# andres-fr/realtime-pose-estimation

Measured on AMD Instinct MI355X. Metric: images/sec at 640x640 (HRNet-w48 fwd+decode), higher is better.
Workload: dtype f16 (fp32 accumulate, fp32 BatchNorm; fp32 NCHW in/out); 1 GPU; configs[2]: batch=32 per GPU, 640x640, half-wrapper teacher forward + decode of 17 keypoint channels, weights W0 (seeded random); batch_per_gpu=32, people_per_batch_rank0=960

## Files before the change

realtime-pose-estimation_amd/csrc/conv_block.hip:

```cpp
#include <type_traits>

#include "rtpe_common.h"

namespace rtpe {

typedef _Float16 half8 __attribute__((ext_vector_type(8)));
typedef _Float16 half4 __attribute__((ext_vector_type(4)));
typedef float float4v __attribute__((ext_vector_type(4)));
typedef float float2v __attribute__((ext_vector_type(2)));
typedef _Float16 half2v __attribute__((ext_vector_type(2)));

__device__ __forceinline__ half4 bn_round(const float4v v, const float4v al, const float4v be) {
  const half2v h0 = __builtin_convertvector(float2v{v[0], v[1]}, half2v);
  const half2v h1 = __builtin_convertvector(float2v{v[2], v[3]}, half2v);
  float r0 = __builtin_fmaf((float)h0[0], al[0], be[0]);
  float r1 = __builtin_fmaf((float)h0[1], al[1], be[1]);
  float r2 = __builtin_fmaf((float)h1[0], al[2], be[2]);
  float r3 = __builtin_fmaf((float)h1[1], al[3], be[3]);
  asm volatile("" : "+v"(r0), "+v"(r1), "+v"(r2), "+v"(r3));
  const half2v o0 = __builtin_convertvector(float2v{r0, r1}, half2v), o1 = __builtin_convertvector(float2v{r2, r3}, half2v);
  return half4{o0[0], o0[1], o1[0], o1[1]};
}
typedef short short8 __attribute__((ext_vector_type(8)));
typedef short short4v __attribute__((ext_vector_type(4)));

namespace {

constexpr int kTH = 6, kTW = 32;
constexpr int kMH = kTH + 2, kMW = kTW + 2;
constexpr int kXH = kTH + 4, kXW = kTW + 4;
constexpr int kPS = 96;
constexpr int kMT = 3;
constexpr int kNT1 = 5, kNT2 = 3;
constexpr int kWaves = 4, kLoad = 3;
constexpr int kKH = 7;
constexpr int kWSlot = kMT * kKH * 1024;
constexpr int kXBytes = kXH * kXW * kPS;
constexpr int kMidBytes = kMH * kMW * kPS;
constexpr int kRowB = kMT * 32 + 16;
constexpr int kNIT = (kNT2 * 16 * 6 + 63) / 64;
constexpr int kLds = 3 * kWSlot + 2 * kXBytes + kMidBytes;

#define RTPE_BBARRIER()                         \
  do {                                          \
    asm volatile("" ::: "memory");              \
    __builtin_amdgcn_s_barrier();               \
    asm volatile("" ::: "memory");              \
  } while (0)

typedef __attribute__((address_space(3))) void* lds_ptr_t;

}

struct BlockArgs {
  const _Float16* x;
  _Float16* y;
  const _Float16* w1;
  const _Float16* w2;
  const float* ab1;
  const float* ab2;
  int N, H, W, in_ld, out_ld;
  int tiles_x, tiles_y;
  FastDiv div_tiles_x, div_tiles_xy;
  int x_bytes;
  int ablate;
};

__global__ void __launch_bounds__((kWaves + kLoad) * 64) conv_block_kernel(const BlockArgs a) {
  extern __shared__ __attribute__((aligned(16))) char smem[];
  char* const wring = smem;
  char* const xt = smem + 3 * kWSlot;
  char* const mid = xt + 2 * kXBytes;
  const int tid = threadIdx.x;
  const int lane = tid & 63;
  const int wv = __builtin_amdgcn_readfirstlane(tid >> 6);

  const int n_tiles = a.N * a.tiles_x * a.tiles_y;
  const int G = (int)(gridDim.x >> 3), xcd = (int)(blockIdx.x & 7), jw = (int)(blockIdx.x >> 3);
  const int per_xcd = (n_tiles + 7) >> 3;
  const int t_begin = xcd * per_xcd;
  const int tiles_xcd = min(per_xcd, n_tiles - t_begin);
  const int U = jw < tiles_xcd ? (tiles_xcd - jw + G - 1) / G : 0;
  if (U == 0) return;
  const uint32_t tiles_xy = (uint32_t)(a.tiles_x * a.tiles_y);
  auto unit_origin = [&](int u, uint32_t* n, int* py0, int* px0) __attribute__((always_inline)) {
    uint32_t t = (uint32_t)(t_begin + jw + u * G);
    *n = fdiv(t, a.div_tiles_xy);
    t -= *n * tiles_xy;
    const uint32_t tyi = fdiv(t, a.div_tiles_x);
    *py0 = (int)tyi * kTH;
    *px0 = (int)(t - tyi * a.tiles_x) * kTW;
  };

  if (wv == kWaves) {
    __amdgpu_buffer_rsrc_t r1 = __builtin_amdgcn_make_buffer_rsrc(const_cast<_Float16*>(a.w1), 0, 2 * kWSlot, 0x00020000);
    __amdgpu_buffer_rsrc_t r2 = __builtin_amdgcn_make_buffer_rsrc(const_cast<_Float16*>(a.w2), 0, 2 * kWSlot, 0x00020000);
    const int voff = lane * 16;
    auto issue = [&](int q) __attribute__((always_inline)) {
      const int i = q & 3;
      char* dst = wring + (q % 3) * kWSlot;
      const int src = (i & 1) * kWSlot;
      if (i < 2) {
#pragma unroll
        for (int p = 0; p < kMT * kKH; ++p)
          __builtin_amdgcn_raw_ptr_buffer_load_lds(r1, (lds_ptr_t)(dst + p * 1024), 16, voff, src + p * 1024, 0, 0);
      } else {
#pragma unroll
        for (int p = 0; p < kMT * kKH; ++p)
          __builtin_amdgcn_raw_ptr_buffer_load_lds(r2, (lds_ptr_t)(dst + p * 1024), 16, voff, src + p * 1024, 0, 0);
      }
    };
    const int Q = 4 * U;
    issue(0);
    issue(1);
    for (int q = 0; q < Q; ++q) {
      if (q + 1 < Q) asm volatile("s_waitcnt vmcnt(%0)" ::"n"(kMT * kKH) : "memory");
      else asm volatile("s_waitcnt vmcnt(0)" ::: "memory");
      RTPE_BBARRIER();
      if (q + 2 < Q) issue(q + 2);
      if ((q & 3) == 3) RTPE_BBARRIER();
    }
    asm volatile("s_waitcnt vmcnt(0)" ::: "memory");
    return;
  }

  if (wv > kWaves) {
    const int jl = wv - kWaves - 1;
    __amdgpu_buffer_rsrc_t rsrc = __builtin_amdgcn_make_buffer_rsrc(const_cast<_Float16*>(a.x), 0, a.x_bytes, 0x00020000);
    constexpr int rowslots = kXW * 6;
    auto issue = [&](int u) __attribute__((always_inline)) {
      uint32_t n;
      int py0, px0;
      unit_origin(u, &n, &py0, &px0);
      const int iy0 = py0 - 2, ix0 = px0 - 2;
      uint32_t voff[4];
#pragma unroll
      for (int k = 0; k < 4; ++k) {
        const int q = k * 64 + lane;
        const int hx = q / 6, sl = q - hx * 6;
        const int ix = ix0 + hx;
        voff[k] = (unsigned)ix < (unsigned)a.W ? (uint32_t)(ix * a.in_ld + sl * 8) * 2u : 0x80000000u;
      }
      char* buf = xt + (u & 1) * kXBytes;
      const int img_row0 = (int)n * a.H;
      for (int r = jl * (kXH / 2); r < (jl + 1) * (kXH / 2); ++r) {
        const int iy = iy0 + r;
        const bool row_ok = (unsigned)iy < (unsigned)a.H;
        const int soff = row_ok ? (img_row0 + iy) * a.W * a.in_ld * 2 : 0;
        char* dst = buf + r * (kXW * kPS);
#pragma unroll
        for (int k = 0; k < 4; ++k)
          if (k * 64 + lane < rowslots)
            __builtin_amdgcn_raw_ptr_buffer_load_lds(rsrc, (lds_ptr_t)(dst + k * 1024), 16,
                                                     (int)(row_ok ? voff[k] : 0x80000000u), soff, 0, 0);
      }
    };
    issue(0);
    for (int u = 0; u < U; ++u) {
      asm volatile("s_waitcnt vmcnt(0)" ::: "memory");
      RTPE_BBARRIER();
      if (u + 1 < U) issue(u + 1);
      RTPE_BBARRIER();
      RTPE_BBARRIER();
      RTPE_BBARRIER();
      RTPE_BBARRIER();
    }
    asm volatile("s_waitcnt vmcnt(0)" ::: "memory");
    return;
  }

  const int r = lane & 15, g = lane >> 4;
  int toff1[2 * kKH], toff2[2 * kKH];
#pragma unroll
  for (int k = 0; k < 2 * kKH; ++k) {
    int kk = k * 32 + g * 8;
    if (kk >= 9 * 48) kk -= 9 * 48;
    const int tap = kk / 48, c = kk - tap * 48;
    const int ty = tap / 3, tx = tap - ty * 3;
    toff1[k] = (ty * kXW + tx) * kPS + c * 2;
    toff2[k] = (ty * kMW + tx) * kPS + c * 2;
  }
  int pix1[kNT1], pix2[kNT2];
#pragma unroll
  for (int nt = 0; nt < kNT1; ++nt) {
    int p = (wv * kNT1 + nt) * 16 + r;
    p = p < kMH * kMW ? p : kMH * kMW - 1;
    const int my = p / kMW, mx = p - my * kMW;
    pix1[nt] = (my * kXW + mx) * kPS;
  }
#pragma unroll
  for (int nt = 0; nt < kNT2; ++nt) {
    const int p = (wv * kNT2 + nt) * 16 + r;
    pix2[nt] = ((p >> 5) * kMW + (p & 31)) * kPS;
  }
  float4v al1[kMT], be1[kMT], al2[kMT], be2[kMT];
#pragma unroll
  for (int m = 0; m < kMT; ++m) {
    const int c4 = m * 16 + g * 4;
    al1[m] = *reinterpret_cast<const float4v*>(a.ab1 + c4);
    be1[m] = *reinterpret_cast<const float4v*>(a.ab1 + 48 + c4);
    al2[m] = *reinterpret_cast<const float4v*>(a.ab2 + c4);
    be2[m] = *reinterpret_cast<const float4v*>(a.ab2 + 48 + c4);
  }
#pragma unroll
  for (int m = 0; m < kMT; ++m) asm volatile("" ::"v"(al1[m]), "v"(be1[m]), "v"(al2[m]), "v"(be2[m]));

  int eoff[kNIT], xoff[kNIT], epos[kNIT];
#pragma unroll
  for (int it = 0; it < kNIT; ++it) {
    int c = it * 64 + lane;
    const bool exists = c < kNT2 * 16 * 6;
    c = exists ? c : 0;
    const int pw = c / 6, slot = c - pw * 6;
    const int p = wv * kNT2 * 16 + pw;
    const int oy = p >> 5, ox = p & 31;
    eoff[it] = pw * kRowB + slot * 16;
    xoff[it] = ((oy + 2) * kXW + ox + 2) * kPS + slot * 16;
    epos[it] = ((exists ? oy : 0x7fff) << 16) | (ox << 8) | (slot * 16);
  }
  int wsel = 0;
  for (int u = 0; u < U; ++u) {
    uint32_t n;
    int py0, px0;
    unit_origin(u, &n, &py0, &px0);
    const char* xb = xt + (u & 1) * kXBytes;

    float4v acc1[kMT][kNT1];
#pragma unroll
    for (int m = 0; m < kMT; ++m)
#pragma unroll
      for (int nt = 0; nt < kNT1; ++nt) acc1[m][nt] = float4v{0.f, 0.f, 0.f, 0.f};
#pragma unroll
    for (int h = 0; h < 2; ++h) {
      RTPE_BBARRIER();
      const char* wl = wring + wsel * kWSlot + lane * 16;
      wsel = wsel == 2 ? 0 : wsel + 1;
      half8 af[2][kMT], bf[2][kNT1];
#pragma unroll
      for (int m = 0; m < kMT; ++m) af[0][m] = *reinterpret_cast<const half8*>(wl + m * 1024);
#pragma unroll
      for (int nt = 0; nt < kNT1; ++nt) bf[0][nt] = *reinterpret_cast<const half8*>(xb + pix1[nt] + toff1[h * kKH]);
#pragma unroll
      for (int kk = 0; kk < kKH; ++kk) {
        const int cur = kk & 1, nxt = cur ^ 1;
        if (kk + 1 < kKH) {
#pragma unroll
          for (int m = 0; m < kMT; ++m) af[nxt][m] = *reinterpret_cast<const half8*>(wl + ((kk + 1) * kMT + m) * 1024);
#pragma unroll
          for (int nt = 0; nt < kNT1; ++nt)
            bf[nxt][nt] = *reinterpret_cast<const half8*>(xb + pix1[nt] + toff1[h * kKH + kk + 1]);
        }
#pragma unroll
        for (int m = 0; m < kMT; ++m)
#pragma unroll
          for (int nt = 0; nt < kNT1; ++nt)
            acc1[m][nt] = __builtin_amdgcn_mfma_f32_16x16x32_f16(af[cur][m], bf[cur][nt], acc1[m][nt], 0, 0, 0);
        if (kk + 1 < kKH) {
#pragma unroll
          for (int i = 0; i < (kMT + kNT1 + 3) / 4; ++i) {
            __builtin_amdgcn_sched_group_barrier(0x008, 1, 0);
            __builtin_amdgcn_sched_group_barrier(0x002, 4, 0);
            __builtin_amdgcn_sched_group_barrier(0x100, 4, 0);
          }
        }
        __builtin_amdgcn_sched_barrier(0);
      }
    }
    {
      int lane_e = lane;
      asm volatile("" : "+v"(lane_e));
      const int re = lane_e & 15, ge = lane_e >> 4;
#pragma unroll
      for (int nt = 0; nt < kNT1; ++nt) {
        const int p = (wv * kNT1 + nt) * 16 + re;
        const int my = p / kMW, mx = p - my * kMW;
        const int iy = py0 - 1 + my, ix = px0 - 1 + mx;
        const bool inside = (unsigned)iy < (unsigned)a.H && (unsigned)ix < (unsigned)a.W;
#pragma unroll
        for (int m = 0; m < kMT; ++m) {
          const half4 o_bn = bn_round(acc1[m][nt], al1[m], be1[m]);
          short4v b = __builtin_bit_cast(short4v, o_bn);
          b = b & ~(b >> 15);
          if (!inside) b = b ^ b;
          if (p < kMH * kMW)
            *reinterpret_cast<short4v*>(mid + p * kPS + m * 32 + ge * 8) = b;
        }
      }
      asm volatile("s_waitcnt lgkmcnt(0)" ::: "memory");
    }

    float4v acc2[kMT][kNT2];
#pragma unroll
    for (int m = 0; m < kMT; ++m)
#pragma unroll
      for (int nt = 0; nt < kNT2; ++nt) acc2[m][nt] = float4v{0.f, 0.f, 0.f, 0.f};
#pragma unroll
    for (int h = 0; h < 2; ++h) {
      RTPE_BBARRIER();
      const char* wl = wring + wsel * kWSlot + lane * 16;
      wsel = wsel == 2 ? 0 : wsel + 1;
      half8 af[2][kMT], bf[2][kNT2];
#pragma unroll
      for (int m = 0; m < kMT; ++m) af[0][m] = *reinterpret_cast<const half8*>(wl + m * 1024);
#pragma unroll
      for (int nt = 0; nt < kNT2; ++nt) bf[0][nt] = *reinterpret_cast<const half8*>(mid + pix2[nt] + toff2[h * kKH]);
#pragma unroll
      for (int kk = 0; kk < kKH; ++kk) {
        const int cur = kk & 1, nxt = cur ^ 1;
        if (kk + 1 < kKH) {
#pragma unroll
          for (int m = 0; m < kMT; ++m) af[nxt][m] = *reinterpret_cast<const half8*>(wl + ((kk + 1) * kMT + m) * 1024);
#pragma unroll
          for (int nt = 0; nt < kNT2; ++nt)
            bf[nxt][nt] = *reinterpret_cast<const half8*>(mid + pix2[nt] + toff2[h * kKH + kk + 1]);
        }
#pragma unroll
        for (int m = 0; m < kMT; ++m)
#pragma unroll
          for (int nt = 0; nt < kNT2; ++nt)
            acc2[m][nt] = __builtin_amdgcn_mfma_f32_16x16x32_f16(af[cur][m], bf[cur][nt], acc2[m][nt], 0, 0, 0);
        if (kk + 1 < kKH) {
#pragma unroll
          for (int i = 0; i < (kMT + kNT2 + 3) / 4; ++i) {
            __builtin_amdgcn_sched_group_barrier(0x008, 1, 0);
            __builtin_amdgcn_sched_group_barrier(0x002, 4, 0);
            __builtin_amdgcn_sched_group_barrier(0x100, 4, 0);
          }
        }
        __builtin_amdgcn_sched_barrier(0);
      }
    }
    {
      int lane_e = lane;
      asm volatile("" : "+v"(lane_e));
      const int re = lane_e & 15, ge = lane_e >> 4;
      asm volatile("s_waitcnt lgkmcnt(0)" ::: "memory");
      RTPE_BBARRIER();
      char* obuf = mid + wv * (kNT2 * 16 * kRowB);
#pragma unroll
      for (int nt = 0; nt < kNT2; ++nt)
#pragma unroll
        for (int m = 0; m < kMT; ++m) {
          const half4 o_bn = bn_round(acc2[m][nt], al2[m], be2[m]);
          *reinterpret_cast<half4*>(obuf + (nt * 16 + re) * kRowB + m * 32 + ge * 8) = o_bn;
        }
      half8 ov[kNIT], rv[kNIT];
#pragma unroll
      for (int it = 0; it < kNIT; ++it) {
        ov[it] = *reinterpret_cast<const half8*>(obuf + eoff[it]);
        rv[it] = *reinterpret_cast<const half8*>(xb + xoff[it]);
      }
      const int hy = a.H - py0, hx = a.W - px0;
      char* const yb = reinterpret_cast<char*>(a.y + (((size_t)n * a.H + py0) * a.W + px0) * a.out_ld);
      const uint32_t ld2 = (uint32_t)a.out_ld * 2u, row_pix = (uint32_t)a.W & 0xffffffu;
#pragma unroll
      for (int it = 0; it < kNIT; ++it) {
        int e = epos[it];
        asm volatile("" : "+v"(e));
        half8 v = ov[it] + rv[it];
        short8 b = __builtin_bit_cast(short8, v);
        b = b & ~(b >> 15);
        if ((e >> 16) < hy && ((e >> 8) & 255) < hx) {
          const uint32_t pix = __umul24((uint32_t)e >> 16, row_pix) + (((uint32_t)e >> 8) & 255u);
          *reinterpret_cast<short8*>(yb + __umul24(pix, ld2) + ((uint32_t)e & 255u)) = b;
        }
      }
      asm volatile("s_waitcnt lgkmcnt(0)" ::: "memory");
    }
  }
}

namespace {
constexpr int kLdsRW = 4 * kWSlot + kXBytes + kMidBytes;
}

__global__ void __launch_bounds__((kWaves + kLoad) * 64) conv_block_rw_kernel(const BlockArgs a) {
  extern __shared__ __attribute__((aligned(16))) char smem[];
  char* const wts = smem;
  char* const xb = smem + 4 * kWSlot;
  char* const mid = xb + kXBytes;
  const int tid = threadIdx.x;
  const int lane = tid & 63;
  const int wv = __builtin_amdgcn_readfirstlane(tid >> 6);

  const int n_tiles = a.N * a.tiles_x * a.tiles_y;
  const int G = (int)(gridDim.x >> 3), xcd = (int)(blockIdx.x & 7), jw = (int)(blockIdx.x >> 3);
  const int per_xcd = (n_tiles + 7) >> 3;
  const int t_begin = xcd * per_xcd;
  const int tiles_xcd = min(per_xcd, n_tiles - t_begin);
  const int U = jw < tiles_xcd ? (tiles_xcd - jw + G - 1) / G : 0;
  if (U == 0) return;
  const uint32_t tiles_xy = (uint32_t)(a.tiles_x * a.tiles_y);
  auto unit_origin = [&](int u, uint32_t* n, int* py0, int* px0) __attribute__((always_inline)) {
    uint32_t t = (uint32_t)(t_begin + jw + u * G);
    *n = fdiv(t, a.div_tiles_xy);
    t -= *n * tiles_xy;
    const uint32_t tyi = fdiv(t, a.div_tiles_x);
    *py0 = (int)tyi * kTH;
    *px0 = (int)(t - tyi * a.tiles_x) * kTW;
  };

  if (wv >= kWaves) {
    const int jl = wv - kWaves;
    const int r0 = jl == 0 ? 0 : jl == 1 ? 4 : 7, r1 = jl == 0 ? 4 : jl == 1 ? 7 : 10;
    __amdgpu_buffer_rsrc_t rsrc = __builtin_amdgcn_make_buffer_rsrc(const_cast<_Float16*>(a.x), 0, a.x_bytes, 0x00020000);
    constexpr int rowslots = kXW * 6;
    auto issue = [&](int u) __attribute__((always_inline)) {
      uint32_t n;
      int py0, px0;
      unit_origin(u, &n, &py0, &px0);
      const int iy0 = py0 - 2, ix0 = px0 - 2;
      uint32_t voff[4];
#pragma unroll
      for (int k = 0; k < 4; ++k) {
        const int q = k * 64 + lane;
        const int hx = q / 6, sl = q - hx * 6;
        const int ix = ix0 + hx;
        voff[k] = (unsigned)ix < (unsigned)a.W ? (uint32_t)(ix * a.in_ld + sl * 8) * 2u : 0x80000000u;
      }
      const int img_row0 = (int)n * a.H;
      for (int r = r0; r < r1; ++r) {
        const int iy = iy0 + r;
        const bool row_ok = (unsigned)iy < (unsigned)a.H;
        const int soff = row_ok ? (img_row0 + iy) * a.W * a.in_ld * 2 : 0;
        char* dst = xb + r * (kXW * kPS);
#pragma unroll
        for (int k = 0; k < 4; ++k)
          if (k * 64 + lane < rowslots)
            __builtin_amdgcn_raw_ptr_buffer_load_lds(rsrc, (lds_ptr_t)(dst + k * 1024), 16,
                                                     (int)(row_ok ? voff[k] : 0x80000000u), soff, 0, 0);
      }
    };
    if (jl < 2) {
      __amdgpu_buffer_rsrc_t rw = __builtin_amdgcn_make_buffer_rsrc(const_cast<_Float16*>(jl == 0 ? a.w1 : a.w2), 0,
                                                                    2 * kWSlot, 0x00020000);
      char* dst = wts + jl * 2 * kWSlot;
      const int voff = lane * 16;
      for (int p = 0; p < 2 * kMT * kKH; ++p)
        __builtin_amdgcn_raw_ptr_buffer_load_lds(rw, (lds_ptr_t)(dst + p * 1024), 16, voff, p * 1024, 0, 0);
    }
    issue(0);
    for (int u = 0; u < U; ++u) {
      asm volatile("s_waitcnt vmcnt(0)" ::: "memory");
      RTPE_BBARRIER();
      RTPE_BBARRIER();
      if (u + 1 < U && !(a.ablate & 1)) issue(u + 1);
      RTPE_BBARRIER();
    }
    asm volatile("s_waitcnt vmcnt(0)" ::: "memory");
    return;
  }

  const int r = lane & 15, g = lane >> 4;
  int b1a[kNT1], b1b[kNT1], b1c[kNT1], b2a[kNT2], b2b[kNT2], b2c[kNT2];
  {
    const int hi = g >= 2 ? 1 : 0;
#pragma unroll
    for (int nt = 0; nt < kNT1; ++nt) {
      int p = (wv * kNT1 + nt) * 16 + r;
      p = p < kMH * kMW ? p : kMH * kMW - 1;
      const int my = p / kMW, mx = p - my * kMW;
      b1a[nt] = (int)(4 * kWSlot) + (my * kXW + mx) * kPS + g * 16;
      b1b[nt] = b1a[nt] + hi * (kXW - 3) * kPS;
      b1c[nt] = b1a[nt] - hi * ((2 * kXW + 2) * kPS + 96);
    }
#pragma unroll
    for (int nt = 0; nt < kNT2; ++nt) {
      const int p = (wv * kNT2 + nt) * 16 + r;
      b2a[nt] = (int)(4 * kWSlot + kXBytes) + ((p >> 5) * kMW + (p & 31)) * kPS + g * 16;
      b2b[nt] = b2a[nt] + hi * (kMW - 3) * kPS;
      b2c[nt] = b2a[nt] - hi * ((2 * kMW + 2) * kPS + 96);
    }
  }
  float4v al1[kMT], be1[kMT], al2[kMT], be2[kMT];
#pragma unroll
  for (int m = 0; m < kMT; ++m) {
    const int c4 = m * 16 + g * 4;
    al1[m] = *reinterpret_cast<const float4v*>(a.ab1 + c4);
    be1[m] = *reinterpret_cast<const float4v*>(a.ab1 + 48 + c4);
    al2[m] = *reinterpret_cast<const float4v*>(a.ab2 + c4);
    be2[m] = *reinterpret_cast<const float4v*>(a.ab2 + 48 + c4);
  }
#pragma unroll
  for (int m = 0; m < kMT; ++m) asm volatile("" ::"v"(al1[m]), "v"(be1[m]), "v"(al2[m]), "v"(be2[m]));

  int eoff[kNIT], xoff[kNIT], epos[kNIT];
#pragma unroll
  for (int it = 0; it < kNIT; ++it) {
    int c = it * 64 + lane;
    const bool exists = c < kNT2 * 16 * 6;
    c = exists ? c : 0;
    const int pw = c / 6, slot = c - pw * 6;
    const int p = wv * kNT2 * 16 + pw;
    const int oy = p >> 5, ox = p & 31;
    eoff[it] = pw * kRowB + slot * 16;
    xoff[it] = ((oy + 2) * kXW + ox + 2) * kPS + slot * 16;
    epos[it] = ((exists ? oy : 0x7fff) << 16) | (ox << 8) | (slot * 16);
  }

  auto kloop = [&](const char* wbase, const int* ba, const int* bb, const int* bc, auto acc, auto ntc, auto pitch)
      __attribute__((always_inline)) {
    constexpr int NT = decltype(ntc)::value, RW = decltype(pitch)::value;
    const char* wl = wbase + lane * 16;
    auto koff = [](int k) constexpr { const int tap = (32 * k) / 48; return ((tap / 3) * RW + tap % 3) * kPS + ((32 * k) % 48) * 2; };
    auto bptr = [&](int k, int nt) __attribute__((always_inline)) {
      const int base = k == 4 ? bb[nt] : k == 13 ? bc[nt] : ba[nt];
      return reinterpret_cast<const half8*>(smem + base + koff(k));
    };
    half8 af[2][kMT], bf[2][NT];
#pragma unroll
    for (int m = 0; m < kMT; ++m) af[0][m] = *reinterpret_cast<const half8*>(wl + m * 1024);
#pragma unroll
    for (int nt = 0; nt < NT; ++nt) bf[0][nt] = *bptr(0, nt);
#pragma unroll
    for (int kk = 0; kk < 2 * kKH; ++kk) {
      const int cur = kk & 1, nxt = cur ^ 1;
      if (kk + 1 < 2 * kKH) {
#pragma unroll
        for (int m = 0; m < kMT; ++m) af[nxt][m] = *reinterpret_cast<const half8*>(wl + ((kk + 1) * kMT + m) * 1024);
#pragma unroll
        for (int nt = 0; nt < NT; ++nt) bf[nxt][nt] = *bptr(kk + 1, nt);
      }
#pragma unroll
      for (int m = 0; m < kMT; ++m)
#pragma unroll
        for (int nt = 0; nt < NT; ++nt)
          acc[m][nt] = __builtin_amdgcn_mfma_f32_16x16x32_f16(af[cur][m], bf[cur][nt], acc[m][nt], 0, 0, 0);
      if (kk + 1 < 2 * kKH) {
#pragma unroll
        for (int i = 0; i < (kMT + NT + 1) / 2; ++i) {
          __builtin_amdgcn_sched_group_barrier(0x008, 1, 0);
          __builtin_amdgcn_sched_group_barrier(0x100, 2, 0);
        }
      }
      __builtin_amdgcn_sched_barrier(0);
    }
  };

  for (int u = 0; u < U; ++u) {
    uint32_t n;
    int py0, px0;
    unit_origin(u, &n, &py0, &px0);

    RTPE_BBARRIER();
    half8 rv[kNIT];
#pragma unroll
    for (int it = 0; it < kNIT; ++it) rv[it] = *reinterpret_cast<const half8*>(xb + xoff[it]);

    float4v acc1[kMT][kNT1];
#pragma unroll
    for (int m = 0; m < kMT; ++m)
#pragma unroll
      for (int nt = 0; nt < kNT1; ++nt) acc1[m][nt] = float4v{0.f, 0.f, 0.f, 0.f};
    if (!(a.ablate & 8)) kloop(wts, b1a, b1b, b1c, acc1, std::integral_constant<int, kNT1>(), std::integral_constant<int, kXW>());
    if (!(a.ablate & 2)) {
      int lane_e = lane;
      asm volatile("" : "+v"(lane_e));
      const int re = lane_e & 15, ge = lane_e >> 4;
#pragma unroll
      for (int nt = 0; nt < kNT1; ++nt) {
        const int p = (wv * kNT1 + nt) * 16 + re;
        const int my = p / kMW, mx = p - my * kMW;
        const int iy = py0 - 1 + my, ix = px0 - 1 + mx;
        const bool inside = (unsigned)iy < (unsigned)a.H && (unsigned)ix < (unsigned)a.W;
#pragma unroll
        for (int m = 0; m < kMT; ++m) {
          const half4 o_bn = bn_round(acc1[m][nt], al1[m], be1[m]);
          short4v b = __builtin_bit_cast(short4v, o_bn);
          b = b & ~(b >> 15);
          if (!inside) b = b ^ b;
          if (p < kMH * kMW)
            *reinterpret_cast<short4v*>(mid + p * kPS + m * 32 + ge * 8) = b;
        }
      }
      asm volatile("s_waitcnt lgkmcnt(0)" ::: "memory");
    }
#pragma unroll
    for (int it = 0; it < kNIT; ++it) asm volatile("" : "+v"(rv[it]));

    RTPE_BBARRIER();
    float4v acc2[kMT][kNT2];
#pragma unroll
    for (int m = 0; m < kMT; ++m)
#pragma unroll
      for (int nt = 0; nt < kNT2; ++nt) acc2[m][nt] = float4v{0.f, 0.f, 0.f, 0.f};
    if (!(a.ablate & 8)) kloop(wts + 2 * kWSlot, b2a, b2b, b2c, acc2, std::integral_constant<int, kNT2>(), std::integral_constant<int, kMW>());
    {
      int lane_e = lane;
      asm volatile("" : "+v"(lane_e));
      const int re = lane_e & 15, ge = lane_e >> 4;
      asm volatile("s_waitcnt lgkmcnt(0)" ::: "memory");
      RTPE_BBARRIER();
      char* obuf = mid + wv * (kNT2 * 16 * kRowB);
#pragma unroll
      for (int nt = 0; nt < kNT2; ++nt)
#pragma unroll
        for (int m = 0; m < kMT; ++m) {
          const half4 o_bn = bn_round(acc2[m][nt], al2[m], be2[m]);
          *reinterpret_cast<half4*>(obuf + (nt * 16 + re) * kRowB + m * 32 + ge * 8) = o_bn;
        }
      half8 ov[kNIT];
#pragma unroll
      for (int it = 0; it < kNIT; ++it) ov[it] = *reinterpret_cast<const half8*>(obuf + eoff[it]);
      const int hy = a.H - py0, hx = a.W - px0;
      char* const yb = reinterpret_cast<char*>(a.y + (((size_t)n * a.H + py0) * a.W + px0) * a.out_ld);
      const uint32_t ld2 = (uint32_t)a.out_ld * 2u, row_pix = (uint32_t)a.W & 0xffffffu;
#pragma unroll
      for (int it = 0; it < kNIT; ++it) {
        int e = epos[it];
        asm volatile("" : "+v"(e));
        half8 v = ov[it] + rv[it];
        short8 b = __builtin_bit_cast(short8, v);
        b = b & ~(b >> 15);
        if ((e >> 16) < hy && ((e >> 8) & 255) < hx && !(a.ablate & 4)) {
          const uint32_t pix = __umul24((uint32_t)e >> 16, row_pix) + (((uint32_t)e >> 8) & 255u);
          *reinterpret_cast<short8*>(yb + __umul24(pix, ld2) + ((uint32_t)e & 255u)) = b;
        }
      }
      asm volatile("s_waitcnt lgkmcnt(0)" ::: "memory");
    }
  }
}

namespace {
constexpr int kPTH = 8, kPTW = 16;
constexpr int kPMH = kPTH + 2, kPMW = kPTW + 2;
constexpr int kPXH = kPTH + 4, kPXW = kPTW + 4;
constexpr int kPNT1 = 3, kPNT2 = 2;
constexpr int kPXRow = 2240;
constexpr int kPMRow = kPMW * kPS;
constexpr int kPXBytes = kPXH * kPXRow;
constexpr int kPMidBytes = kPMH * kPMRow;
constexpr int kPObuf = kPNT2 * 16 * kRowB;
constexpr int kPOffX = 2 * kWSlot;
constexpr int kPOffMid = kPOffX + 2 * kPXBytes;
constexpr int kPOffObuf = kPOffMid + 2 * kPMidBytes;
constexpr int kPOffBn = kPOffObuf + 4 * kPObuf;
constexpr int kPOffRes = kPOffBn + 96 * 4;
constexpr int kLdsPC = kPOffRes + 4 * 3072;
constexpr int kPNIT = kPNT2 * 16 * 6 / 64;
static_assert(kPXW * 6 <= 128 && kPXRow >= 128 * 16, "an x-tile row is two full-wave requests");
static_assert(kPMH * kPMW <= 4 * kPNT1 * 16, "conv1 region fits the producers' column tiles");
}

#ifdef RTPE_DIAG
__device__ unsigned long long g_pc_trace[8 * 64];
#define RTPE_PC_TRACE(slot)                                                                                     \
  do {                                                                                                          \
    if (trace_on && (slot) < 64) {                                                                              \
      const unsigned long long t_ = __builtin_amdgcn_s_memrealtime();                                             \
      if (lane == 0) *reinterpret_cast<volatile unsigned long long*>(smem + kLdsPC + (wv * 64 + (slot)) * 8) = t_; \
    }                                                                                                           \
  } while (0)
#define RTPE_PC_TRACE_FLUSH()                                                                                   \
  do {                                                                                                          \
    if (trace_on) g_pc_trace[wv * 64 + lane] = *reinterpret_cast<unsigned long long*>(smem + kLdsPC + (wv * 64 + lane) * 8); \
  } while (0)
#else
#define RTPE_PC_TRACE(slot) do { } while (0)
#define RTPE_PC_TRACE_FLUSH() do { } while (0)
#endif

__global__ void __launch_bounds__(512) conv_block_pc_kernel(const BlockArgs a) {
  extern __shared__ __attribute__((aligned(16))) char smem[];
  const int tid = threadIdx.x;
  const int lane = tid & 63;
  const int wv = __builtin_amdgcn_readfirstlane(tid >> 6);

  const int n_tiles = a.N * a.tiles_x * a.tiles_y;
  const int G = (int)(gridDim.x >> 3), xcd = (int)(blockIdx.x & 7), jw = (int)(blockIdx.x >> 3);
  const int per_xcd = (n_tiles + 7) >> 3;
  const int t_begin = xcd * per_xcd;
  const int tiles_xcd = min(per_xcd, n_tiles - t_begin);
  const int U = jw < tiles_xcd ? (tiles_xcd - jw + G - 1) / G : 0;
  if (U == 0) return;
#ifdef RTPE_DIAG
  const bool trace_on = blockIdx.x == 8 * 3 + 2 && a.H == 160;
  if (trace_on) *reinterpret_cast<unsigned long long*>(smem + kLdsPC + tid * 8) = 0ull;
#endif
  const uint32_t tiles_xy = (uint32_t)(a.tiles_x * a.tiles_y);
  auto unit_origin = [&](int u, uint32_t* n, int* py0, int* px0) __attribute__((always_inline)) {
    uint32_t t = (uint32_t)(t_begin + jw + u * G);
    *n = fdiv(t, a.div_tiles_xy);
    t -= *n * tiles_xy;
    const uint32_t tyi = fdiv(t, a.div_tiles_x);
    *py0 = (int)tyi * kPTH;
    *px0 = (int)(t - tyi * a.tiles_x) * kPTW;
  };
  const int r = lane & 15, g = lane >> 4;
  const int hi = g >= 2 ? 1 : 0;
  auto koff = [](int k, int rowb) constexpr { const int tap = (32 * k) / 48; return (tap / 3) * rowb + (tap % 3) * kPS + ((32 * k) % 48) * 2; };

  __amdgpu_buffer_rsrc_t rsrc = __builtin_amdgcn_make_buffer_rsrc(const_cast<_Float16*>(a.x), 0, a.x_bytes, 0x00020000);
  const int wq = wv & 3;
  int xcol[2];
  uint32_t xoffs[2];
#pragma unroll
  for (int k = 0; k < 2; ++k) {
    const int q = k * 64 + lane;
    const int hx = q / 6, sl = q - hx * 6;
    xcol[k] = q < kPXW * 6 ? hx - 2 : -(1 << 20);
    xoffs[k] = (uint32_t)((hx - 2) * a.in_ld + sl * 8) * 2u;
  }
  struct XReq { uint32_t voff[2][kPXH / 4]; int soff[kPXH / 4]; };
  auto prepare_x = [&](int u, XReq& q) __attribute__((always_inline)) {
    uint32_t n;
    int py0, px0;
    unit_origin(u, &n, &py0, &px0);
    const int iy0 = py0 - 2 + wq * (kPXH / 4);
    uint32_t voff[2];
#pragma unroll
    for (int k = 0; k < 2; ++k)
      voff[k] = (unsigned)(px0 + xcol[k]) < (unsigned)a.W ? xoffs[k] + (uint32_t)(px0 * a.in_ld) * 2u : 0x80000000u;
    const int img_row0 = (int)n * a.H;
#pragma unroll
    for (int j = 0; j < kPXH / 4; ++j) {
      const int iy = iy0 + j;
      const bool row_ok = (unsigned)iy < (unsigned)a.H;
      q.soff[j] = row_ok ? (img_row0 + iy) * a.W * a.in_ld * 2 : 0;
#pragma unroll
      for (int k = 0; k < 2; ++k) q.voff[k][j] = row_ok ? voff[k] : 0x80000000u;
    }
  };
  auto fire_x = [&](const XReq& q, int par) __attribute__((always_inline)) {
    char* buf = smem + kPOffX + par * kPXBytes + wq * (kPXH / 4) * kPXRow;
#pragma unroll
    for (int j = 0; j < kPXH / 4; ++j)
#pragma unroll
      for (int k = 0; k < 2; ++k)
        __builtin_amdgcn_raw_ptr_buffer_load_lds(rsrc, (lds_ptr_t)(buf + j * kPXRow + k * 1024), 16, (int)q.voff[k][j],
                                                 q.soff[j], 0, 0);
  };
  auto issue_x = [&](int u, int par) __attribute__((always_inline)) {
    XReq q;
    prepare_x(u, q);
    fire_x(q, par);
  };

  if (wv < 4) {
    int ba[kPNT1], bb[kPNT1], bc[kPNT1];
#pragma unroll
    for (int nt = 0; nt < kPNT1; ++nt) {
      int p = (wv * kPNT1 + nt) * 16 + r;
      p = p < kPMH * kPMW ? p : kPMH * kPMW - 1;
      const int my = p / kPMW, mx = p - my * kPMW;
      ba[nt] = kPOffX + my * kPXRow + mx * kPS + g * 16;
      bb[nt] = ba[nt] + hi * (kPXRow - 3 * kPS);
      bc[nt] = ba[nt] - hi * (2 * kPXRow + 2 * kPS + 96);
    }
    int moff[kPNT1], myx[kPNT1];
#pragma unroll
    for (int nt = 0; nt < kPNT1; ++nt) {
      int p = (wv * kPNT1 + nt) * 16 + r;
      p = p < kPMH * kPMW ? p : kPMH * kPMW - 1;
      moff[nt] = p * kPS + g * 8;
      myx[nt] = ((p / kPMW) << 8) | (p % kPMW);
    }
    float4v al1[kMT], be1[kMT];
#pragma unroll
    for (int m = 0; m < kMT; ++m) {
      const int c4 = m * 16 + g * 4;
      al1[m] = *reinterpret_cast<const float4v*>(a.ab1 + c4);
      be1[m] = *reinterpret_cast<const float4v*>(a.ab1 + 48 + c4);
    }
#pragma unroll
    for (int m = 0; m < kMT; ++m) asm volatile("" : "+v"(al1[m]), "+v"(be1[m]));
    const char* wl = smem + lane * 16;
    for (int i = 0; i < U; ++i) {
      uint32_t n;
      int py0, px0;
      unit_origin(i, &n, &py0, &px0);
      const int xsel = (i & 1) * kPXBytes;
      XReq xq;
      prepare_x(i + 1 < U ? i + 1 : U - 1, xq);
#pragma unroll
      for (int j = 0; j < kPXH / 4; ++j) asm volatile("" : "+v"(xq.voff[0][j]), "+v"(xq.voff[1][j]), "+s"(xq.soff[j]));
      RTPE_PC_TRACE(i * 5 + 0);
      RTPE_BBARRIER();
      RTPE_PC_TRACE(i * 5 + 1);
      RTPE_PC_TRACE(i * 5 + 2);
      float4v acc[kMT][kPNT1];
#pragma unroll
      for (int m = 0; m < kMT; ++m)
#pragma unroll
        for (int nt = 0; nt < kPNT1; ++nt) acc[m][nt] = float4v{0.f, 0.f, 0.f, 0.f};
      if (!(a.ablate & 4)) {
        const char* ta[kPNT1];
        const char* tb[kPNT1];
        const char* tc[kPNT1];
#pragma unroll
        for (int nt = 0; nt < kPNT1; ++nt) {
          ta[nt] = smem + ba[nt] + xsel; tb[nt] = smem + bb[nt] + xsel; tc[nt] = smem + bc[nt] + xsel;
        }
        auto bptr = [&](int k, int nt) __attribute__((always_inline)) {
          return reinterpret_cast<const half8*>((k == 4 ? tb[nt] : k == 13 ? tc[nt] : ta[nt]) + koff(k, kPXRow));
        };
        half8 af[3][kMT], bf[3][kPNT1];
#pragma unroll
        for (int s0 = 0; s0 < 2; ++s0) {
#pragma unroll
          for (int m = 0; m < kMT; ++m) af[s0][m] = *reinterpret_cast<const half8*>(wl + (s0 * kMT + m) * 1024);
#pragma unroll
          for (int nt = 0; nt < kPNT1; ++nt) bf[s0][nt] = *bptr(s0, nt);
        }
#pragma unroll
        for (int kk = 0; kk < 2 * kKH; ++kk) {
          const int cur = kk % 3, nxt = (kk + 2) % 3;
          if (kk + 2 < 2 * kKH) {
#pragma unroll
            for (int m = 0; m < kMT; ++m) af[nxt][m] = *reinterpret_cast<const half8*>(wl + ((kk + 2) * kMT + m) * 1024);
#pragma unroll
            for (int nt = 0; nt < kPNT1; ++nt) bf[nxt][nt] = *bptr(kk + 2, nt);
          }
#pragma unroll
          for (int m = 0; m < kMT; ++m)
#pragma unroll
            for (int nt = 0; nt < kPNT1; ++nt)
              acc[m][nt] = __builtin_amdgcn_mfma_f32_16x16x32_f16(af[cur][m], bf[cur][nt], acc[m][nt], 0, 0, 0);
          if (kk + 2 < 2 * kKH) {
#pragma unroll
            for (int q = 0; q < kMT + kPNT1; ++q) {
              __builtin_amdgcn_sched_group_barrier(0x008, 1, 0);
              __builtin_amdgcn_sched_group_barrier(0x100, 1, 0);
            }
          }
          __builtin_amdgcn_sched_barrier(0);
        }
      }
#ifdef RTPE_DIAG
      if (!(a.ablate & 32))
#endif
      fire_x(xq, (i + 1) & 1);
      RTPE_PC_TRACE(i * 5 + 3);
      if (!(a.ablate & 1)) {
        char* mid = smem + kPOffMid + (i & 1) * kPMidBytes;
        const bool interior = py0 >= 1 && py0 + kPTH < a.H && px0 >= 1 && px0 + kPTW < a.W;
        auto bn_relu = [&](int m, int nt) __attribute__((always_inline)) {
          const float4v v = acc[m][nt];
          half4 o = bn_round(v, al1[m], be1[m]);
          short4v b = __builtin_bit_cast(short4v, o);
          return b & ~(b >> 15);
        };
        if (interior) {
#pragma unroll
          for (int nt = 0; nt < kPNT1; ++nt)
#pragma unroll
            for (int m = 0; m < kMT; ++m) *reinterpret_cast<short4v*>(mid + moff[nt] + m * 32) = bn_relu(m, nt);
        } else {
#pragma unroll
          for (int nt = 0; nt < kPNT1; ++nt) {
            const int iy = py0 - 1 + (myx[nt] >> 8), ix = px0 - 1 + (myx[nt] & 255);
            const bool inside = (unsigned)iy < (unsigned)a.H && (unsigned)ix < (unsigned)a.W;
#pragma unroll
            for (int m = 0; m < kMT; ++m) {
              short4v b = bn_relu(m, nt);
              if (!inside) b = b ^ b;
              *reinterpret_cast<short4v*>(mid + moff[nt] + m * 32) = b;
            }
          }
        }
        asm volatile("s_waitcnt lgkmcnt(0)" ::: "memory");
      }
      RTPE_PC_TRACE(i * 5 + 4);
      asm volatile("s_waitcnt vmcnt(0)" ::: "memory");
    }
    RTPE_PC_TRACE(U * 5 < 60 ? U * 5 : 60);
    RTPE_BBARRIER();
    RTPE_PC_TRACE_FLUSH();
    return;
  }

  const int cw = wv - 4;
  {
    __amdgpu_buffer_rsrc_t rw = __builtin_amdgcn_make_buffer_rsrc(const_cast<_Float16*>(a.w1), 0, 2 * kWSlot, 0x00020000);
    const int voff = lane * 16;
    for (int p = cw; p < 2 * kMT * kKH; p += 4)
      __builtin_amdgcn_raw_ptr_buffer_load_lds(rw, (lds_ptr_t)(smem + p * 1024), 16, voff, p * 1024, 0, 0);
    if (cw == 0 && lane < 24) reinterpret_cast<float4*>(smem + kPOffBn)[lane] = reinterpret_cast<const float4*>(a.ab2)[lane];
  }
  issue_x(0, 0);
  half8 w2[2 * kKH][kMT];
#pragma unroll
  for (int k = 0; k < 2 * kKH; ++k)
#pragma unroll
    for (int m = 0; m < kMT; ++m)
      w2[k][m] = *reinterpret_cast<const half8*>(reinterpret_cast<const char*>(a.w2) + ((k * kMT + m) * 64 + lane) * 16);
  int ca[kPNT2];
#pragma unroll
  for (int nt = 0; nt < kPNT2; ++nt)
    ca[nt] = kPOffMid + ((cw * kPNT2 + nt) * kPMW + r) * kPS + g * 16;
  const int hi4 = hi * (kPMRow - 3 * kPS), hi13 = -hi * (2 * kPMRow + 2 * kPS + 96);
  uint32_t ooffs[kPNIT], xoffr[kPNIT], yoffr[kPNIT];
#pragma unroll
  for (int it = 0; it < kPNIT; ++it) {
    const int c = it * 64 + lane;
    const int pw = c / 6, slot = c - pw * 6;
    ooffs[it] = (uint32_t)(pw * kRowB + slot * 16);
    xoffr[it] = (uint32_t)(((pw >> 4) * a.W + (pw & 15)) * a.in_ld * 2 + slot * 16);
    yoffr[it] = (uint32_t)(((pw >> 4) * a.W + (pw & 15)) * a.out_ld * 2 + slot * 16);
  }
  asm volatile("s_waitcnt vmcnt(0)" ::: "memory");
#pragma unroll
  for (int k = 0; k < 2 * kKH; ++k)
#pragma unroll
    for (int m = 0; m < kMT; ++m) asm volatile("" : "+v"(w2[k][m]));
  asm volatile("s_waitcnt lgkmcnt(0)" ::: "memory");

  float4v acc[kMT][kPNT2];
  auto conv2 = [&](int v) __attribute__((always_inline)) {
    const int msel = (v & 1) * kPMidBytes;
#pragma unroll
    for (int m = 0; m < kMT; ++m)
#pragma unroll
      for (int nt = 0; nt < kPNT2; ++nt) acc[m][nt] = float4v{0.f, 0.f, 0.f, 0.f};
    if (a.ablate & 8) return;
    const char* ta[kPNT2];
#pragma unroll
    for (int nt = 0; nt < kPNT2; ++nt) ta[nt] = smem + ca[nt] + msel;
    auto bptr = [&](int k, int nt) __attribute__((always_inline)) {
      return reinterpret_cast<const half8*>(ta[nt] + (k == 4 ? hi4 : k == 13 ? hi13 : 0) + koff(k, kPMRow));
    };
    half8 bf[3][kPNT2];
#pragma unroll
    for (int s0 = 0; s0 < 2; ++s0)
#pragma unroll
      for (int nt = 0; nt < kPNT2; ++nt) bf[s0][nt] = *bptr(s0, nt);
#pragma unroll
    for (int kk = 0; kk < 2 * kKH; ++kk) {
      const int cur = kk % 3, nxt = (kk + 2) % 3;
      if (kk + 2 < 2 * kKH) {
#pragma unroll
        for (int nt = 0; nt < kPNT2; ++nt) bf[nxt][nt] = *bptr(kk + 2, nt);
      }
#pragma unroll
      for (int m = 0; m < kMT; ++m)
#pragma unroll
        for (int nt = 0; nt < kPNT2; ++nt)
          acc[m][nt] = __builtin_amdgcn_mfma_f32_16x16x32_f16(w2[kk][m], bf[cur][nt], acc[m][nt], 0, 0, 0);
      if (kk + 2 < 2 * kKH) {
#pragma unroll
        for (int q = 0; q < kPNT2; ++q) {
          __builtin_amdgcn_sched_group_barrier(0x008, 1, 0);
          __builtin_amdgcn_sched_group_barrier(0x100, 1, 0);
        }
      }
      __builtin_amdgcn_sched_barrier(0);
    }
  };
  struct Bn2 { float4v al[kMT], be[kMT]; };
  auto load_bn = [&](Bn2& bn) __attribute__((always_inline)) {
#pragma unroll
    for (int m = 0; m < kMT; ++m) {
      bn.al[m] = *reinterpret_cast<const float4v*>(smem + kPOffBn + (m * 16 + g * 4) * 4);
      bn.be[m] = *reinterpret_cast<const float4v*>(smem + kPOffBn + (48 + m * 16 + g * 4) * 4);
    }
  };
  char* const res = smem + kPOffRes + cw * 3072;
  auto request_residual = [&](int v) __attribute__((always_inline)) -> char* {
    uint32_t n;
    int py0, px0;
    unit_origin(v, &n, &py0, &px0);
    const int pix0 = ((int)n * a.H + py0 + cw * kPNT2) * a.W + px0;
#pragma unroll
    for (int it = 0; it < kPNIT; ++it)
      __builtin_amdgcn_raw_ptr_buffer_load_lds(rsrc, (lds_ptr_t)(res + it * 1024), 16, (int)xoffr[it], pix0 * a.in_ld * 2, 0, 0);
    return reinterpret_cast<char*>(a.y + (size_t)pix0 * a.out_ld);
  };
  auto epilogue = [&](const Bn2& bn, char* yb) __attribute__((always_inline)) {
    int lane_e = lane;
    asm volatile("" : "+v"(lane_e));
    const int re = lane_e & 15, ge = lane_e >> 4;
    char* obuf = smem + kPOffObuf + cw * kPObuf;
#pragma unroll
    for (int m = 0; m < kMT; ++m) {
      const float4v al = bn.al[m], be = bn.be[m];
#pragma unroll
      for (int nt = 0; nt < kPNT2; ++nt) {
        *reinterpret_cast<half4*>(obuf + (nt * 16 + re) * kRowB + m * 32 + ge * 8) = bn_round(acc[m][nt], al, be);
      }
    }
    asm volatile("s_waitcnt vmcnt(0)" ::: "memory");
#pragma unroll
    for (int it = 0; it < kPNIT; ++it) {
      const half8 ov = *reinterpret_cast<const half8*>(obuf + ooffs[it]);
      const half8 rv = *reinterpret_cast<const half8*>(res + it * 1024 + lane_e * 16);
      half8 o = ov + rv;
      short8 b = __builtin_bit_cast(short8, o);
      b = b & ~(b >> 15);
      store16_wt(yb + yoffr[it], b);
    }
    asm volatile("s_waitcnt lgkmcnt(0)" ::: "memory");
  };

  RTPE_BBARRIER();
  Bn2 bn;
  char* yb_next = nullptr;
  if (U > 1) {
    RTPE_BBARRIER();
    yb_next = request_residual(0);
    conv2(0);
    load_bn(bn);
    asm volatile("s_waitcnt lgkmcnt(0)" ::: "memory");
  }
  for (int i = 2; i <= U; ++i) {
    RTPE_PC_TRACE((i - 2) * 5 + 0);
    RTPE_BBARRIER();
    RTPE_PC_TRACE((i - 2) * 5 + 1);
    char* const yb = yb_next;
    epilogue(bn, yb);
    RTPE_PC_TRACE((i - 2) * 5 + 2);
    yb_next = request_residual(i - 1);
    RTPE_PC_TRACE((i - 2) * 5 + 3);
    conv2(i - 1);
    RTPE_PC_TRACE((i - 2) * 5 + 4);
    load_bn(bn);
    asm volatile("s_waitcnt lgkmcnt(0)" ::: "memory");
  }
  {
    if (U == 1) {
      RTPE_BBARRIER();
      yb_next = request_residual(0);
      conv2(0);
      load_bn(bn);
    }
    epilogue(bn, yb_next);
  }
  RTPE_PC_TRACE_FLUSH();
}


bool conv_block_supports(int cin, int cout, int H, int W) { return cin == 48 && cout == 48 && H >= kTH && W >= 16; }

int conv_block_launch(const _Float16* x, int in_ld, size_t x_bytes, _Float16* y, int out_ld, const _Float16* w1,
                      const float* ab1, const _Float16* w2, const float* ab2, int N, int H, int W, hipStream_t s) {
  RTPE_REQUIRE(x && y && w1 && w2 && ab1 && ab2 && N > 0, "basic block: null argument");
  RTPE_REQUIRE(in_ld % 8 == 0 && out_ld % 8 == 0 && in_ld >= 48 && out_ld >= 48 && (((uintptr_t)x | (uintptr_t)y) & 15) == 0,
               "basic block: NHWC views must be 16-byte aligned (in_ld=%d out_ld=%d)", in_ld, out_ld);
  RTPE_REQUIRE(x_bytes > 0 && x_bytes < 0x80000000ull, "basic block: input view of %zu bytes", x_bytes);
  const int ring = get_option(kOptBlockRing);
  const bool pc = get_option(kOptBlockPC) != 0 && !ring && H % kPTH == 0 && W % kPTW == 0;
  static unsigned long long attr_mask = 0;
  if (first_use_on_device(&attr_mask)) {
    RTPE_HIP_CHECK(hipFuncSetAttribute(reinterpret_cast<const void*>(conv_block_kernel),
                                       hipFuncAttributeMaxDynamicSharedMemorySize, 160 * 1024));
    RTPE_HIP_CHECK(hipFuncSetAttribute(reinterpret_cast<const void*>(conv_block_rw_kernel),
                                       hipFuncAttributeMaxDynamicSharedMemorySize, 160 * 1024));
    RTPE_HIP_CHECK(hipFuncSetAttribute(reinterpret_cast<const void*>(conv_block_pc_kernel),
                                       hipFuncAttributeMaxDynamicSharedMemorySize, 160 * 1024));
  }
  BlockArgs a;
  memset(&a, 0, sizeof(a));
  a.x = x; a.y = y; a.w1 = w1; a.w2 = w2; a.ab1 = ab1; a.ab2 = ab2;
  a.N = N; a.H = H; a.W = W; a.in_ld = in_ld; a.out_ld = out_ld;
  a.tiles_x = pc ? W / kPTW : (W + kTW - 1) / kTW;
  a.tiles_y = pc ? H / kPTH : (H + kTH - 1) / kTH;
  a.div_tiles_x = make_fastdiv(a.tiles_x);
  a.div_tiles_xy = make_fastdiv(a.tiles_x * a.tiles_y);
  a.x_bytes = (int)x_bytes;
  static const int abl = RTPE_DIAG_ENV_INT("RTPE_BLOCK_ABL", 0);
  a.ablate = abl;
  const long tiles = (long)N * a.tiles_x * a.tiles_y;
  static const int g_env = env_int("RTPE_PERSIST_G", 32);
  long G = g_env;
  if (G > (tiles + 7) / 8) G = (tiles + 7) / 8;
  if (pc)
#ifdef RTPE_DIAG
    hipLaunchKernelGGL(conv_block_pc_kernel, dim3((unsigned)(8 * G)), dim3(512), kLdsPC + 8 * 64 * 8, s, a);
#else
    hipLaunchKernelGGL(conv_block_pc_kernel, dim3((unsigned)(8 * G)), dim3(512), kLdsPC, s, a);
#endif
  else if (ring)
    hipLaunchKernelGGL(conv_block_kernel, dim3((unsigned)(8 * G)), dim3((kWaves + kLoad) * 64), kLds, s, a);
  else
    hipLaunchKernelGGL(conv_block_rw_kernel, dim3((unsigned)(8 * G)), dim3((kWaves + kLoad) * 64), kLdsRW, s, a);
  RTPE_HIP_CHECK(hipGetLastError());
  return RTPE_OK;
}

}

#ifdef RTPE_DIAG
extern "C" int rtpe_diag_pc_trace(unsigned long long* out) {
  return hipMemcpyFromSymbol(out, HIP_SYMBOL(rtpe::g_pc_trace), sizeof(unsigned long long) * 8 * 64) == hipSuccess ? 0 : -1;
}
#endif
```

Measured before the change: 2397 images/sec.

## Keep W1 in producer registers and move x-tile prefetch to conv2 waves

Compiles the ablation checks out unless RTPE_DIAG is defined, so the non-diagnostic build no longer tests a runtime ablate mask in the hot loops. In the producer/consumer kernel, the first eight k-steps of the conv1 weights are preloaded into registers, which removes their per-tile LDS reads. With the default request mode, the next x tile is no longer fetched by the conv1 producer waves; the conv2 waves issue it alongside the residual request and wait for it after conv2. The aim is to take LDS traffic and load issue off the conv1 critical path, at the cost of more VGPRs in the producers and a new split of synchronisation between the two wave groups.

After: 2394 images/sec. Within noise of the previous version (-0.1%).

```diff
diff --git a/realtime-pose-estimation_amd/csrc/conv_block.hip b/realtime-pose-estimation_amd/csrc/conv_block.hip
--- a/realtime-pose-estimation_amd/csrc/conv_block.hip
+++ b/realtime-pose-estimation_amd/csrc/conv_block.hip
@@ -65,6 +65,12 @@
   int x_bytes;
   int ablate;
 };
+
+#ifdef RTPE_DIAG
+#define RTPE_BLOCK_ABL(bit) (a.ablate & (bit))
+#else
+#define RTPE_BLOCK_ABL(bit) 0
+#endif
 
 __global__ void __launch_bounds__((kWaves + kLoad) * 64) conv_block_kernel(const BlockArgs a) {
   extern __shared__ __attribute__((aligned(16))) char smem[];
@@ -444,7 +450,7 @@
       asm volatile("s_waitcnt vmcnt(0)" ::: "memory");
       RTPE_BBARRIER();
       RTPE_BBARRIER();
-      if (u + 1 < U && !(a.ablate & 1)) issue(u + 1);
+      if (u + 1 < U && !RTPE_BLOCK_ABL(1)) issue(u + 1);
       RTPE_BBARRIER();
     }
     asm volatile("s_waitcnt vmcnt(0)" ::: "memory");
@@ -552,8 +558,8 @@
     for (int m = 0; m < kMT; ++m)
 #pragma unroll
       for (int nt = 0; nt < kNT1; ++nt) acc1[m][nt] = float4v{0.f, 0.f, 0.f, 0.f};
-    if (!(a.ablate & 8)) kloop(wts, b1a, b1b, b1c, acc1, std::integral_constant<int, kNT1>(), std::integral_constant<int, kXW>());
-    if (!(a.ablate & 2)) {
+    if (!RTPE_BLOCK_ABL(8)) kloop(wts, b1a, b1b, b1c, acc1, std::integral_constant<int, kNT1>(), std::integral_constant<int, kXW>());
+    if (!RTPE_BLOCK_ABL(2)) {
       int lane_e = lane;
       asm volatile("" : "+v"(lane_e));
       const int re = lane_e & 15, ge = lane_e >> 4;
@@ -584,7 +590,7 @@
     for (int m = 0; m < kMT; ++m)
 #pragma unroll
       for (int nt = 0; nt < kNT2; ++nt) acc2[m][nt] = float4v{0.f, 0.f, 0.f, 0.f};
-    if (!(a.ablate & 8)) kloop(wts + 2 * kWSlot, b2a, b2b, b2c, acc2, std::integral_constant<int, kNT2>(), std::integral_constant<int, kMW>());
+    if (!RTPE_BLOCK_ABL(8)) kloop(wts + 2 * kWSlot, b2a, b2b, b2c, acc2, std::integral_constant<int, kNT2>(), std::integral_constant<int, kMW>());
     {
       int lane_e = lane;
       asm volatile("" : "+v"(lane_e));
@@ -612,7 +618,7 @@
         half8 v = ov[it] + rv[it];
         short8 b = __builtin_bit_cast(short8, v);
         b = b & ~(b >> 15);
-        if ((e >> 16) < hy && ((e >> 8) & 255) < hx && !(a.ablate & 4)) {
+        if ((e >> 16) < hy && ((e >> 8) & 255) < hx && !RTPE_BLOCK_ABL(4)) {
           const uint32_t pix = __umul24((uint32_t)e >> 16, row_pix) + (((uint32_t)e >> 8) & 255u);
           *reinterpret_cast<short8*>(yb + __umul24(pix, ld2) + ((uint32_t)e & 255u)) = b;
         }
@@ -639,6 +645,19 @@
 constexpr int kPOffRes = kPOffBn + 96 * 4;
 constexpr int kLdsPC = kPOffRes + 4 * 3072;
 constexpr int kPNIT = kPNT2 * 16 * 6 / 64;
+#ifndef RTPE_PC_W1REG
+#define RTPE_PC_W1REG 8
+#endif
+#ifndef RTPE_PC_XREQ
+#define RTPE_PC_XREQ 2
+#endif
+#ifndef RTPE_PC_XREQ_K
+#define RTPE_PC_XREQ_K 10
+#endif
+constexpr int kPW1R = RTPE_PC_W1REG;
+constexpr int kPXReq = RTPE_PC_XREQ, kPXReqK = RTPE_PC_XREQ_K;
+static_assert(kPW1R >= 0 && kPW1R <= 2 * kKH, "k-steps of W1 in producer registers");
+static_assert(kPXReq >= 0 && kPXReq <= 2 && kPXReqK >= 0 && kPXReqK < 2 * kKH, "x-tile request form");
 static_assert(kPXW * 6 <= 128 && kPXRow >= 128 * 16, "an x-tile row is two full-wave requests");
 static_assert(kPMH * kPMW <= 4 * kPNT1 * 16, "conv1 region fits the producers' column tiles");
 }
@@ -722,10 +741,10 @@
       for (int k = 0; k < 2; ++k) q.voff[k][j] = row_ok ? voff[k] : 0x80000000u;
     }
   };
-  auto fire_x = [&](const XReq& q, int par) __attribute__((always_inline)) {
+  auto fire_x = [&](const XReq& q, int par, int j0 = 0, int j1 = kPXH / 4) __attribute__((always_inline)) {
     char* buf = smem + kPOffX + par * kPXBytes + wq * (kPXH / 4) * kPXRow;
 #pragma unroll
-    for (int j = 0; j < kPXH / 4; ++j)
+    for (int j = j0; j < j1; ++j)
 #pragma unroll
       for (int k = 0; k < 2; ++k)
         __builtin_amdgcn_raw_ptr_buffer_load_lds(rsrc, (lds_ptr_t)(buf + j * kPXRow + k * 1024), 16, (int)q.voff[k][j],
@@ -766,15 +785,28 @@
 #pragma unroll
     for (int m = 0; m < kMT; ++m) asm volatile("" : "+v"(al1[m]), "+v"(be1[m]));
     const char* wl = smem + lane * 16;
+    half8 w1r[kPW1R > 0 ? kPW1R : 1][kMT];
+#pragma unroll
+    for (int k = 0; k < kPW1R; ++k)
+#pragma unroll
+      for (int m = 0; m < kMT; ++m)
+        w1r[k][m] = *reinterpret_cast<const half8*>(reinterpret_cast<const char*>(a.w1) + ((k * kMT + m) * 64 + lane) * 16);
+    asm volatile("s_waitcnt vmcnt(0)" ::: "memory");
+#pragma unroll
+    for (int k = 0; k < kPW1R; ++k)
+#pragma unroll
+      for (int m = 0; m < kMT; ++m) asm volatile("" : "+v"(w1r[k][m]));
     for (int i = 0; i < U; ++i) {
       uint32_t n;
       int py0, px0;
       unit_origin(i, &n, &py0, &px0);
       const int xsel = (i & 1) * kPXBytes;
       XReq xq;
-      prepare_x(i + 1 < U ? i + 1 : U - 1, xq);
-#pragma unroll
-      for (int j = 0; j < kPXH / 4; ++j) asm volatile("" : "+v"(xq.voff[0][j]), "+v"(xq.voff[1][j]), "+s"(xq.soff[j]));
+      if (kPXReq < 2) {
+        prepare_x(i + 1 < U ? i + 1 : U - 1, xq);
+#pragma unroll
+        for (int j = 0; j < kPXH / 4; ++j) asm volatile("" : "+v"(xq.voff[0][j]), "+v"(xq.voff[1][j]), "+s"(xq.soff[j]));
+      }
       RTPE_PC_TRACE(i * 5 + 0);
       RTPE_BBARRIER();
       RTPE_PC_TRACE(i * 5 + 1);
@@ -784,7 +816,7 @@
       for (int m = 0; m < kMT; ++m)
 #pragma unroll
         for (int nt = 0; nt < kPNT1; ++nt) acc[m][nt] = float4v{0.f, 0.f, 0.f, 0.f};
-      if (!(a.ablate & 4)) {
+      if (!RTPE_BLOCK_ABL(4)) {
         const char* ta[kPNT1];
         const char* tb[kPNT1];
         const char* tc[kPNT1];
@@ -798,17 +830,23 @@
         half8 af[3][kMT], bf[3][kPNT1];
 #pragma unroll
         for (int s0 = 0; s0 < 2; ++s0) {
-#pragma unroll
-          for (int m = 0; m < kMT; ++m) af[s0][m] = *reinterpret_cast<const half8*>(wl + (s0 * kMT + m) * 1024);
+          if (s0 >= kPW1R) {
+#pragma unroll
+            for (int m = 0; m < kMT; ++m) af[s0][m] = *reinterpret_cast<const half8*>(wl + (s0 * kMT + m) * 1024);
+          }
 #pragma unroll
           for (int nt = 0; nt < kPNT1; ++nt) bf[s0][nt] = *bptr(s0, nt);
         }
 #pragma unroll
         for (int kk = 0; kk < 2 * kKH; ++kk) {
           const int cur = kk % 3, nxt = (kk + 2) % 3;
+          const bool fetch_a = kk + 2 >= kPW1R;
+          if (kPXReq == 1 && kk == kPXReqK && !RTPE_BLOCK_ABL(32)) fire_x(xq, (i + 1) & 1, 0, 1);
           if (kk + 2 < 2 * kKH) {
-#pragma unroll
-            for (int m = 0; m < kMT; ++m) af[nxt][m] = *reinterpret_cast<const half8*>(wl + ((kk + 2) * kMT + m) * 1024);
+            if (fetch_a) {
+#pragma unroll
+              for (int m = 0; m < kMT; ++m) af[nxt][m] = *reinterpret_cast<const half8*>(wl + ((kk + 2) * kMT + m) * 1024);
+            }
 #pragma unroll
             for (int nt = 0; nt < kPNT1; ++nt) bf[nxt][nt] = *bptr(kk + 2, nt);
           }
@@ -816,10 +854,11 @@
           for (int m = 0; m < kMT; ++m)
 #pragma unroll
             for (int nt = 0; nt < kPNT1; ++nt)
-              acc[m][nt] = __builtin_amdgcn_mfma_f32_16x16x32_f16(af[cur][m], bf[cur][nt], acc[m][nt], 0, 0, 0);
+              acc[m][nt] = __builtin_amdgcn_mfma_f32_16x16x32_f16(kk < kPW1R ? w1r[kk < kPW1R ? kk : 0][m] : af[cur][m],
+                                                                  bf[cur][nt], acc[m][nt], 0, 0, 0);
           if (kk + 2 < 2 * kKH) {
 #pragma unroll
-            for (int q = 0; q < kMT + kPNT1; ++q) {
+            for (int q = 0; q < (fetch_a ? kMT : 0) + kPNT1; ++q) {
               __builtin_amdgcn_sched_group_barrier(0x008, 1, 0);
               __builtin_amdgcn_sched_group_barrier(0x100, 1, 0);
             }
@@ -827,12 +866,10 @@
           __builtin_amdgcn_sched_barrier(0);
         }
       }
-#ifdef RTPE_DIAG
-      if (!(a.ablate & 32))
-#endif
-      fire_x(xq, (i + 1) & 1);
+      if (kPXReq < 2 && !RTPE_BLOCK_ABL(32))
+        fire_x(xq, (i + 1) & 1, kPXReq == 1 ? 1 : 0);
       RTPE_PC_TRACE(i * 5 + 3);
-      if (!(a.ablate & 1)) {
+      if (!RTPE_BLOCK_ABL(1)) {
         char* mid = smem + kPOffMid + (i & 1) * kPMidBytes;
         const bool interior = py0 >= 1 && py0 + kPTH < a.H && px0 >= 1 && px0 + kPTW < a.W;
         auto bn_relu = [&](int m, int nt) __attribute__((always_inline)) {
@@ -862,7 +899,7 @@
         asm volatile("s_waitcnt lgkmcnt(0)" ::: "memory");
       }
       RTPE_PC_TRACE(i * 5 + 4);
-      asm volatile("s_waitcnt vmcnt(0)" ::: "memory");
+      if (kPXReq < 2) asm volatile("s_waitcnt vmcnt(0)" ::: "memory");
     }
     RTPE_PC_TRACE(U * 5 < 60 ? U * 5 : 60);
     RTPE_BBARRIER();
@@ -913,7 +950,7 @@
     for (int m = 0; m < kMT; ++m)
 #pragma unroll
       for (int nt = 0; nt < kPNT2; ++nt) acc[m][nt] = float4v{0.f, 0.f, 0.f, 0.f};
-    if (a.ablate & 8) return;
+    if (RTPE_BLOCK_ABL(8)) return;
     const char* ta[kPNT2];
 #pragma unroll
     for (int nt = 0; nt < kPNT2; ++nt) ta[nt] = smem + ca[nt] + msel;
@@ -992,15 +1029,26 @@
     asm volatile("s_waitcnt lgkmcnt(0)" ::: "memory");
   };
 
+  auto request_x = [&](int i) __attribute__((always_inline)) {
+    if (kPXReq >= 2 && !RTPE_BLOCK_ABL(32)) issue_x(i + 1 < U ? i + 1 : U - 1, (i + 1) & 1);
+  };
+  auto x_landed = [&]() __attribute__((always_inline)) {
+    if (kPXReq >= 2) asm volatile("s_waitcnt vmcnt(0)" ::: "memory");
+  };
+
   RTPE_BBARRIER();
   Bn2 bn;
   char* yb_next = nullptr;
   if (U > 1) {
+    request_x(0);
+    x_landed();
     RTPE_BBARRIER();
     yb_next = request_residual(0);
+    request_x(1);
     conv2(0);
     load_bn(bn);
     asm volatile("s_waitcnt lgkmcnt(0)" ::: "memory");
+    x_landed();
   }
   for (int i = 2; i <= U; ++i) {
     RTPE_PC_TRACE((i - 2) * 5 + 0);
@@ -1010,11 +1058,13 @@
     epilogue(bn, yb);
     RTPE_PC_TRACE((i - 2) * 5 + 2);
     yb_next = request_residual(i - 1);
+    request_x(i);
     RTPE_PC_TRACE((i - 2) * 5 + 3);
     conv2(i - 1);
     RTPE_PC_TRACE((i - 2) * 5 + 4);
     load_bn(bn);
     asm volatile("s_waitcnt lgkmcnt(0)" ::: "memory");
+    x_landed();
   }
   {
     if (U == 1) {
```
